# computations/root_digger

Measured on AMD Instinct MI355X. Metric: candidate-root lnL evals/sec, higher is better.
Workload: dtype f64

## Files before the change

### root_digger_amd/csrc/kernels_fused.hip

```cpp
#include <algorithm>
#include <cstdlib>

#include "common.hpp"
#include "expm_k4.hpp"
#include "fused.hpp"

namespace rdamd {

#pragma clang fp contract(off)

__device__ __forceinline__ double pow2_neg256(int d) {
  return d == 0 ? 1.0 : (d == 1 ? kScaleThreshold
       : (d == 2 ? kScaleThreshold * kScaleThreshold
       : (d == 3 ? kScaleThreshold * kScaleThreshold * kScaleThreshold : 0.0)));
}

__device__ __forceinline__ unsigned uni(unsigned x) {
  return (unsigned)__builtin_amdgcn_readfirstlane((int)x);
}

template <int TR>
constexpr unsigned tab_doubles() { return 8u * TR; }

typedef unsigned v2u __attribute__((ext_vector_type(2)));
// ... 503 lines not shown
    const unsigned k3 = kind & 3u;                                                              \
    if (k3 == kFusedTT) {                                                                       \
      if (TR == 16) {                                                                           \
        ((lds_f64_ptr)(size_t)tab_wr)[0] = ex;                                                  \
        ((lds_f64_ptr)(size_t)tab_wr)[4 * TR] = ey;                                             \
      } else {    \
        __builtin_amdgcn_s_waitcnt(0x0f70);                                       \
      }                                                                                         \
      RDAMD_STAMP(1)                                                                            \
      _Pragma("unroll") for (int q = 0; q < NS; ++q) { read_row<0, TR>(rowx[q], tx[q]); read_row<kYSlot, TR>(rowy[q], ty[q]); } \
      RDAMD_LOAD_TIPS(nxt, ncx, ncy, nex, ney) RDAMD_LATE_DESC(cur, idx2)                       \
      RDAMD_STAMP(2)                                                                            \
      if (kind & 0x100u) {           \
        if (kind & 0x200u) {     \
          _Pragma("unroll") for (int q = 0; q < NS; ++q) {                                      \
            matvec(M, st.v[q], s0[q]);                                                          \
            if (!SPEC) s0sc[q] = st.sc[q];                                                      \
          }                                                                                     \
        } else if (RL >= 2 && (kind & 0x800u)) {                   \
          _Pragma("unroll") for (int q = 0; q < NS; ++q) {                                      \
            matvec(M, st.v[q], s1[q]);                                                          \
            if (!SPEC) s1sc[q] = st.sc[q];                                                      \
          }                                                                                     \
        } else {                                                                                \
          _Pragma("unroll") for (int q = 0; q < NS; ++q) {                                      \
            double tp[4];                                                                       \
            matvec(M, st.v[q], tp);                                                             \
            if (SP > 0) {                                                                       \
              stack_push<NS, !SPEC>(sp, kind, q, stk_lds, stksc_lds, spill_off, tp, st.sc[q]);  \
            } else {                                                                            \
              double2 *d = stk + (size_t)(sp * NS + q) * 128;                                   \
              d[0] = make_double2(tp[0], tp[1]);                                                \
              d[64] = make_double2(tp[2], tp[3]);                                               \
              if (!SPEC) stk_sc[(sp * NS + q) * 64] = st.sc[q];                                 \
            }                                                                                   \
          }                                                                                     \
          if (SP == 0 || !(kind & 0x20000u)) ++sp;    \
        }                                                                                       \
      }                                                                                         \
      RDAMD_STAMP(3)                                                                            \
      RDAMD_LOAD_M(nxt, M)                                                                      \
      _Pragma("unroll") for (int q = 0; q < NS; ++q) {                                          \
        st.sc[q] = 0;                                                                           \
        if (tt_safe) { _Pragma("unroll") for (int k = 0; k < 4; ++k) st.v[q][k] = tx[q][k] * ty[q][k]; } \
      }                                                                                         \
      if (!tt_safe) combine_sites<NS>(tx, ty, st.v, st.sc);                                     \
    } else if (k3 == kFusedRT) {                                                                \
      if (TR == 16) ((lds_f64_ptr)(size_t)tab_wr)[4 * TR] = ey;                                 \
      else __builtin_amdgcn_s_waitcnt(0x0f70);             \
      RDAMD_STAMP(1)                                                                            \
      _Pragma("unroll") for (int q = 0; q < NS; ++q) read_row<kYSlot, TR>(rowy[q], ty[q]);      \
      RDAMD_LOAD_TIPS(nxt, ncx, ncy, nex, ney) RDAMD_LATE_DESC(cur, idx2)                       \
      RDAMD_STAMP(2)                                                                            \
      _Pragma("unroll") for (int q = 0; q < NS; ++q) matvec(M, st.v[q], tx[q]);                 \
      RDAMD_STAMP(3)                                                                            \
      RDAMD_LOAD_M(nxt, M)                                                                      \
      combine_sites<NS, kRT>(tx, ty, st.v, st.sc);                                          \
    } else {         \
      if (kind & 0x400u) {           \
        RDAMD_STAMP(1)                                                                          \
        RDAMD_LOAD_TIPS(nxt, ncx, ncy, nex, ney) RDAMD_LATE_DESC(cur, idx2)                     \
        RDAMD_STAMP(2)                                                                          \
        _Pragma("unroll") for (int q = 0; q < NS; ++q) matvec(M, st.v[q], tx[q]);               \
        RDAMD_STAMP(3)                                                                          \
        RDAMD_LOAD_M(nxt, M)                                                                    \
        if (!SPEC) { _Pragma("unroll") for (int q = 0; q < NS; ++q) st.sc[q] += s0sc[q]; }      \
        combine_sites<NS, kRP>(tx, s0, st.v, st.sc);                                                 \
      } else if (RL >= 2 && (kind & 0x1000u)) {                                                 \
        RDAMD_STAMP(1)                                                                          \
        RDAMD_LOAD_TIPS(nxt, ncx, ncy, nex, ney) RDAMD_LATE_DESC(cur, idx2)                     \
        RDAMD_STAMP(2)                                                                          \
        _Pragma("unroll") for (int q = 0; q < NS; ++q) matvec(M, st.v[q], tx[q]);               \
        RDAMD_STAMP(3)                                                                          \
        RDAMD_LOAD_M(nxt, M)                                                                    \
        if (!SPEC) { _Pragma("unroll") for (int q = 0; q < NS; ++q) st.sc[q] += s1sc[q]; }      \
        combine_sites<NS, kRP>(tx, s1, st.v, st.sc);                                                 \
      } else {                                                                                  \
        int scy[NS];                                                                            \
        f64x2_t plo[NS], phi[NS];                                                               \
        if (SP == 0 || !(kind & 0x40000u)) --sp;                                                \
        _Pragma("unroll") for (int q = 0; q < NS; ++q) {                                        \
          if (SP > 0) {          \
            stack_pop_issue<NS, !SPEC>(sp, kind, q, stk_lds, stksc_lds, spill_off, plo[q], phi[q], scy[q]); \
          } else {                                                                              \
            const double2 *d = stk + (size_t)(sp * NS + q) * 128;                               \
            const double2 lo = d[0], hi = d[64];                                                \
            ty[q][0] = lo.x; ty[q][1] = lo.y; ty[q][2] = hi.x; ty[q][3] = hi.y;                 \
            scy[q] = SPEC ? 0 : stk_sc[(sp * NS + q) * 64];                                     \
          }                                                                                     \
        }                                                                                       \
        RDAMD_STAMP(1)                                                                          \
        RDAMD_LOAD_TIPS(nxt, ncx, ncy, nex, ney) RDAMD_LATE_DESC(cur, idx2)                     \
        RDAMD_STAMP(2)                                                                          \
        _Pragma("unroll") for (int q = 0; q < NS; ++q) matvec(M, st.v[q], tx[q]);               \
        RDAMD_STAMP(3)                                                                          \
        RDAMD_LOAD_M(nxt, M)                                                                    \
        if (SP > 0) {                                                                           \
          stack_pop_wait<NS, !SPEC>(plo, phi, scy);                                             \
          _Pragma("unroll") for (int q = 0; q < NS; ++q) {                                      \
            ty[q][0] = plo[q].x; ty[q][1] = plo[q].y; ty[q][2] = phi[q].x; ty[q][3] = phi[q].y; \
          }                                                                                     \
        }                                                                                       \
        if (!SPEC) { _Pragma("unroll") for (int q = 0; q < NS; ++q) st.sc[q] += scy[q]; }       \
        combine_sites<NS, kRP>(tx, ty, st.v, st.sc);                                        \
      }                                                                                         \
    }                                                                                           \
    RDAMD_STAMP(4)                                                                              \
    RDAMD_STAMP_STORE(kind)                                                                     \
    if (EXPORT && (kind & 0x18000u)) {     \
      double *ec = (kind & 0x8000u) ? a.export_clv[0] : a.export_clv[1];                        \
      unsigned *en = (kind & 0x8000u) ? a.export_cnt[0] : a.export_cnt[1];                      \
      _Pragma("unroll") for (int q = 0; q < NS; ++q)                                            \
        if (valid[q]) {                                                                         \
          const size_t at = (size_t)site[q] * R + r;                                            \
          reinterpret_cast<double2 *>(ec + at * 4)[0] = make_double2(st.v[q][0], st.v[q][1]);   \
          reinterpret_cast<double2 *>(ec + at * 4)[1] = make_double2(st.v[q][2], st.v[q][3]);   \
          en[at] = (unsigned)st.sc[q];                                                          \
        }                                                                                       \
    }                                                                                           \
  }

    double s0[NS][4];
    int s0sc[NS];
    double s1[NS][4];
    int s1sc[NS];
#pragma unroll
    for (int q = 0; q < NS; ++q) {
      s0sc[q] = 0;
#pragma unroll
      for (int k = 0; k < 4; ++k) s0[q][k] = 0.0;
    }
#pragma unroll
    for (int q = 0; q < NS; ++q) {
      s1sc[q] = 0;
#pragma unroll
      for (int k = 0; k < 4; ++k) s1[q][k] = 0.0;
    }
    FusedOp dA = load_const(prog);
    FusedOp dB = load_const(prog + 1);
    unsigned cxA[NS], cyA[NS], cxB[NS], cyB[NS];
    double exA = 0.5, eyA = 0.25, exB = 0.5, eyB = 0.25;
#pragma unroll
    for (int q = 0; q < NS; ++q) { cxA[q] = cxB[q] = 1; cyA[q] = cyB[q] = 2; }
    RDAMD_LOAD_TIPS_NOW(dA, cxA, cyA, exA, eyA)
#if defined(RDAMD_ABLATION) && defined(RDAMD_ABL_NOTIPS)
#pragma unroll
    for (int q = 0; q < NS; ++q) { cxB[q] = cxA[q]; cyB[q] = cyA[q]; }
#endif
    double M[16];
    RDAMD_LOAD_M(dA, M)
    unsigned i = 0;
    for (; i + 1 < nops; i += 2) {
      RDAMD_STEP(dA, dB, cxA, cyA, exA, eyA, cxB, cyB, exB, eyB, i + 2)
      RDAMD_STEP(dB, dA, cxB, cyB, exB, eyB, cxA, cyA, exA, eyA, i + 3)
    }
    if (i < nops) {
      RDAMD_STEP(dA, dB, cxA, cyA, exA, eyA, cxB, cyB, exB, eyB, i + 2)
    }
#undef RDAMD_STEP
    const double w = rw[r];
#pragma unroll
    for (int q = 0; q < NS; ++q) {
      double f = __builtin_fma(st.v[q][3], freqs[3],
                               __builtin_fma(st.v[q][2], freqs[2], __builtin_fma(st.v[q][1], freqs[1], st.v[q][0] * freqs[0])));
      f *= w;
      if (RW) {
        term[q] = f;
        smin[q] = st.sc[q];
      } else if (r == 0) {
        term[q] = f;
        smin[q] = st.sc[q];
      } else if (st.sc[q] >= smin[q]) {
        term[q] = __builtin_fma(f, pow2_neg256(st.sc[q] - smin[q]), term[q]);
      } else {
        term[q] = __builtin_fma(term[q], pow2_neg256(smin[q] - st.sc[q]), f);
        smin[q] = st.sc[q];
      }
    }
  }

  if (TR > 16) __builtin_amdgcn_s_waitcnt(0x0f70);
  if (RW) {
    __syncthreads();
    double *xf = lds + (size_t)wave * NS * 64 + lane;
    int *xs = reinterpret_cast<int *>(lds + (size_t)R * NS * 64) + (size_t)wave * NS * 64 + lane;
#pragma unroll
    for (int q = 0; q < NS; ++q) {
      xf[q * 64] = term[q];
      xs[q * 64] = smin[q];
    }
    __syncthreads();
    if (wave != 0u) return;
    for (unsigned r = 1; r < R; ++r) {
      const double *yf = lds + (size_t)r * NS * 64 + lane;
      const int *ys = reinterpret_cast<const int *>(lds + (size_t)R * NS * 64) + (size_t)r * NS * 64 + lane;
#pragma unroll
      for (int q = 0; q < NS; ++q) {
        const double f = yf[q * 64];
        const int sc = ys[q * 64];
        if (sc >= smin[q]) {
          term[q] = __builtin_fma(f, pow2_neg256(sc - smin[q]), term[q]);
        } else {
          term[q] = __builtin_fma(term[q], pow2_neg256(smin[q] - sc), f);
          smin[q] = sc;
        }
      }
    }
  }
  if constexpr (SPEC) {
    bool low = false;
#pragma unroll
    for (int q = 0; q < NS; ++q) low = low || (valid[q] && (unsigned)__double2hiint(term[q]) < 0x07B00000u);
    if (__builtin_amdgcn_ballot_w64(low) != 0ull && lane == 0) {
      const_cast<FusedJob *>(a.jobs)[job].tt_unsafe = 1u;
      *a.any_unsafe = 1u;
    }
  }
#pragma unroll
  for (int q = 0; q < NS; ++q) {
    double l = __builtin_fma((double)smin[q], kLogScaleThreshold, log(term[q]));
    l *= (double)a.pattern_weights[site[q]];
    if (!valid[q]) l = 0.0;
    if (a.persite && valid[q]) a.persite[(size_t)job * S + site[q]] = l;
#pragma unroll
    for (int off = 32; off > 0; off >>= 1) l += __shfl_down(l, off);
    if (lane == 0) a.partials[(size_t)job * (gridDim.x * NS) + bx * NS + q] = l;
  }
}

#pragma clang fp contract(fast)

__global__ void __launch_bounds__(256)
fused_finish_kernel(const double *__restrict__ partials, unsigned per_job,
                    const FusedJob *__restrict__ jobs, unsigned unsafe_pass,
                    double *__restrict__ out, double *__restrict__ host_out,
                    const unsigned *__restrict__ any_unsafe, unsigned *__restrict__ host_flag,
                    double *__restrict__ flag_f64) {
  __shared__ double lds[4];
  if (host_flag && blockIdx.x == 0 && threadIdx.x == 0) *host_flag = *any_unsafe;
  if (flag_f64 && blockIdx.x == 0 && threadIdx.x == 0) *flag_f64 = *any_unsafe ? 1.0 : 0.0;
  if ((jobs[blockIdx.x].tt_unsafe != 0u) != (unsafe_pass != 0u)) return;
  const double *p = partials + (size_t)blockIdx.x * per_job;
  double acc = 0.0;
  for (unsigned i = threadIdx.x; i < per_job; i += 256) acc += p[i];
#pragma unroll
  for (int off = 32; off > 0; off >>= 1) acc += __shfl_down(acc, off);
  if ((threadIdx.x & 63) == 0) lds[threadIdx.x >> 6] = acc;
  __syncthreads();
  if (threadIdx.x == 0) {
    const double v = ((lds[0] + lds[1]) + lds[2]) + lds[3];
    out[blockIdx.x] = v;
    if (host_out) host_out[blockIdx.x] = v;
  }
}

struct ExportFixupArgs {
  double *clv[2];
  const unsigned *cnt[2];
  unsigned *scaler[2];
  unsigned sites, R;
};
__global__ void __launch_bounds__(64)
fused_export_fixup_kernel(ExportFixupArgs x) {
  const unsigned k = blockIdx.y;
  double *__restrict__ clv = x.clv[k];
  const unsigned *__restrict__ cnt = x.cnt[k];
  if (!clv) return;
  const unsigned R = x.R;
  for (unsigned site = blockIdx.x * 1024u + threadIdx.x; site < min(x.sites, (blockIdx.x + 1) * 1024u); site += 64u) {
  unsigned smin = cnt[(size_t)site * R];
  for (unsigned r = 1; r < R; ++r) smin = min(smin, cnt[(size_t)site * R + r]);
  for (unsigned r = 0; r < R; ++r) {
    const unsigned d = cnt[(size_t)site * R + r] - smin;
    if (d) {
      const double f = d < 4u ? pow2_neg256((int)d) : (d == 4u ? 0x1p-1024 : 0.0);
      double *v = clv + ((size_t)site * R + r) * 4;
#pragma unroll
      for (int i = 0; i < 4; ++i) v[i] *= f;
    }
  }
  x.scaler[k][site] = smin;
  }
}

__global__ void __launch_bounds__(64)
fused_finish_wave_kernel(const double *__restrict__ partials, unsigned per_job, double *__restrict__ out,
                         double *__restrict__ host_out) {
  double acc[4] = {0.0, 0.0, 0.0, 0.0};
#pragma unroll
  for (unsigned w = 0; w < 4; ++w)
    for (unsigned i = w * 64u + threadIdx.x; i < per_job; i += 256) acc[w] += partials[i];
#pragma unroll
  for (unsigned w = 0; w < 4; ++w)
#pragma unroll
    for (int off = 32; off > 0; off >>= 1) acc[w] += __shfl_down(acc[w], off);
  if (threadIdx.x == 0) {
    const double v = ((acc[0] + acc[1]) + acc[2]) + acc[3];
    out[0] = v;
    if (host_out) host_out[0] = v;
  }
}

constexpr unsigned kSlimPasses = 16;
__global__ void __launch_bounds__(64)
fused_pmatrix_k4_kernel(const double *__restrict__ q, const double *__restrict__ rates,
                        FusedJob *__restrict__ jobs, unsigned n_jobs,
                        unsigned n_mat, unsigned R, double *__restrict__ pmat,
                        double *__restrict__ tiptab, size_t pmat_job_stride, size_t tiptab_job_stride,
                        unsigned table_rows, unsigned *__restrict__ any_unsafe) {
  const unsigned lane = threadIdx.x, e = lane & 15u;
  const int base = (int)(lane & ~15u);
  const size_t per_job = (size_t)n_mat * R;
  const size_t total = per_job * n_jobs;
  for (unsigned pass = 0; pass < kSlimPasses; ++pass) {
    const size_t first = (size_t)blockIdx.x * (kSlimPasses * 4) + pass * 4;
    if (first >= total) break;
    const size_t gid_raw = first + (lane >> 4);
    const bool live = gid_raw < total;
    const size_t gid = live ? gid_raw : total - 1;
    const unsigned job = (unsigned)(gid / per_job);
    const unsigned rem = (unsigned)(gid % per_job);
    const unsigned m = rem / R, r = rem % R;
    const double t = jobs[job].brlen[m] * rates[(size_t)job * R + r];
    double v = expm_k4_coop16(q + (size_t)job * 16, t);
    v = v <= 0.0 ? 0.0 : v;
    if (live) pmat[(size_t)job * pmat_job_stride + ((size_t)m * R + r) * 16 + e] = v;
    double *tt = tiptab + (size_t)job * tiptab_job_stride + ((size_t)m * R + r) * 64;
#pragma unroll
    for (unsigned k = 0; k < 4; ++k) {
      const unsigned L = e + 16u * k;
      const unsigned c = table_rows > 16 ? (L >> 1) & 15u : L >> 2;
      const unsigned i = table_rows > 16 ? (L >> 5) * 2 + (L & 1u) : L & 3u;
      double acc = 0.0;
#pragma unroll
      for (int j = 0; j < 4; ++j) {
        const double pj = __shfl(v, base + (int)i * 4 + j);
        if ((c >> j) & 1) acc += pj;
      }
      if (live) tt[L] = acc;
    }
    if (live && v > 0.0 && v < 0x1p-128) {
      jobs[job].tt_unsafe = 1u;
      *any_unsafe = 1u;
    }
  }
}

__global__ void __launch_bounds__(64)
fused_pmatrix_k4_wide_kernel(const double *__restrict__ q, const double *__restrict__ rates,
                        FusedJob *__restrict__ jobs, unsigned n_jobs,
                        unsigned n_mat, unsigned R, double *__restrict__ pmat,
                        double *__restrict__ tiptab, size_t pmat_job_stride, size_t tiptab_job_stride,
                        unsigned table_rows, unsigned *__restrict__ any_unsafe) {
  __shared__ double sh[64 * 17];
  __shared__ unsigned long long base_pm[64], base_tt[64];
  const unsigned lane = threadIdx.x;
  const size_t per_job = (size_t)n_mat * R;
  const size_t total = per_job * n_jobs;
  const size_t gid_raw = (size_t)blockIdx.x * blockDim.x + threadIdx.x;
  const bool live = gid_raw < total;
  const size_t gid = live ? gid_raw : total - 1;
  const unsigned job = (unsigned)(gid / per_job);
  const unsigned rem = (unsigned)(gid % per_job);
  const unsigned m = rem / R, r = rem % R;
  const double t = jobs[job].brlen[m] * rates[(size_t)job * R + r];
  const double *qq = q + (size_t)job * 16;
  double out[16];
  expm_k4(qq, t, out);
#pragma unroll
  for (int i = 0; i < 16; ++i) {
    out[i] = out[i] <= 0.0 ? 0.0 : out[i];
    sh[lane * 17 + i] = out[i];
  }
  base_pm[lane] = (unsigned long long)job * pmat_job_stride + ((size_t)m * R + r) * 16;
  base_tt[lane] = (unsigned long long)job * tiptab_job_stride + ((size_t)m * R + r) * 64;
  __syncthreads();
  const unsigned n_live = (unsigned)(total - (size_t)blockIdx.x * 64 < 64 ? total - (size_t)blockIdx.x * 64 : 64);
#pragma unroll 4
  for (unsigned it = 0; it < 16; ++it) {
    const unsigned e = it * 64 + lane, pr = e >> 4, k = e & 15u;
    if (pr < n_live) pmat[base_pm[pr] + k] = sh[pr * 17 + k];
  }
  const unsigned c = table_rows > 16 ? (lane >> 1) & 15u : lane >> 2;
  const unsigned i = table_rows > 16 ? (lane >> 5) * 2 + (lane & 1u) : lane & 3u;
  for (unsigned pr = 0; pr < n_live; ++pr) {
    const double *o = sh + pr * 17 + i * 4;
    double acc = 0.0;
#pragma unroll
    for (int j = 0; j < 4; ++j)
      if ((c >> j) & 1) acc += o[j];
    tiptab[base_tt[pr] + lane] = acc;
  }
  bool tiny = false;
#pragma unroll
  for (int k = 0; k < 16; ++k) tiny = tiny || (out[k] > 0.0 && out[k] < 0x1p-128);
  if (tiny) {
    jobs[job].tt_unsafe = 1u;
    *any_unsafe = 1u;
  }
}

hipError_t launch_fused_pmatrix(const FusedArgs &a, const double *d_q, const double *d_rates,
                                unsigned n_jobs, unsigned n_mat, bool slim, hipStream_t stream) {
  const size_t total = (size_t)n_jobs * n_mat * a.rate_cats;
  if (!total) return hipSuccess;
  if (slim)
    fused_pmatrix_k4_kernel<<<(unsigned)((total + kSlimPasses * 4 - 1) / (kSlimPasses * 4)), 64, 0, stream>>>(
        d_q, d_rates, const_cast<FusedJob *>(a.jobs), n_jobs, n_mat, a.rate_cats, const_cast<double *>(a.pmat),
        const_cast<double *>(a.tiptab), a.pmat_job_stride, a.tiptab_job_stride, a.table_rows, a.any_unsafe);
  else
    fused_pmatrix_k4_wide_kernel<<<(unsigned)((total + 63) / 64), 64, 0, stream>>>(
        d_q, d_rates, const_cast<FusedJob *>(a.jobs), n_jobs, n_mat, a.rate_cats, const_cast<double *>(a.pmat),
        const_cast<double *>(a.tiptab), a.pmat_job_stride, a.tiptab_job_stride, a.table_rows, a.any_unsafe);
  return hipGetLastError();
}

template <int NS, bool TTCHECK, int RL, int TR, bool RW, int SP, bool EXPORT = false, bool SPEC = false>
static hipError_t launch_fused_variant(const FusedArgs &a, unsigned n_jobs, unsigned max_depth, unsigned gx,
                                       hipStream_t stream) {
  const unsigned n_waves = RW ? a.rate_cats : 1u;
  const size_t per_wave = tab_doubles<TR>() * sizeof(double) +
                          (size_t)(SP > 0 || !max_depth ? 1 : max_depth) * NS * 64 * (4 * sizeof(double) + sizeof(int));
  const size_t lds = std::max<size_t>(per_wave * n_waves, (size_t)n_waves * NS * 64 * 12);
  {
    static std::mutex lds_mu;
    static size_t lds_allowed = 48 * 1024;
    std::lock_guard<std::mutex> guard(lds_mu);
    if (lds > lds_allowed) {
      hipError_t e = hipFuncSetAttribute((const void *)fused_dna_eval_kernel<NS, TTCHECK, RL, TR, RW, SP, EXPORT, SPEC>,
                                         hipFuncAttributeMaxDynamicSharedMemorySize, (int)lds);
      if (e != hipSuccess) return e;
      lds_allowed = lds;
    }
  }
  static const bool lds_starts_at_zero = [] {
    hipFuncAttributes attr;
    return hipFuncGetAttributes(&attr, (const void *)fused_dna_eval_kernel<NS, TTCHECK, RL, TR, RW, SP, EXPORT, SPEC>) == hipSuccess &&
           attr.sharedSizeBytes == 0;
  }();
  if (!lds_starts_at_zero) return hipErrorInvalidValue;
  fused_dna_eval_kernel<NS, TTCHECK, RL, TR, RW, SP, EXPORT, SPEC><<<dim3(gx, a.job_major ? (n_jobs + 7u) / 8u * 8u : n_jobs), 64 * n_waves, lds, stream>>>(a);
  return hipGetLastError();
}

template <int NS, bool TTCHECK, int TR>
static hipError_t launch_fused_variant_rl(const FusedArgs &a, unsigned n_jobs, unsigned max_depth, unsigned gx,
                                          unsigned reg_levels, hipStream_t stream) {
#ifdef RDAMD_ABLATION
  static const unsigned spill_min = getenv("RDAMD_FUSED_SPILL_MIN") ? (unsigned)atoi(getenv("RDAMD_FUSED_SPILL_MIN")) : 2u;
#else
  constexpr unsigned spill_min = 2u;
#endif
  const bool spill = TR > 16 && reg_levels < 2 && max_depth >= spill_min && max_depth <= kFusedSpillLevels;
  if (a.rates_across_waves) {
    if (spill) return launch_fused_variant<NS, TTCHECK, 1, TR, true, kFusedSpillLevels>(a, n_jobs, max_depth, gx, stream);
    return reg_levels >= 2 ? launch_fused_variant<NS, TTCHECK, 2, TR, true, 0>(a, n_jobs, max_depth, gx, stream)
                           : launch_fused_variant<NS, TTCHECK, 1, TR, true, 0>(a, n_jobs, max_depth, gx, stream);
  }
  if constexpr (!TTCHECK)
    if (a.speculate) {
      if (spill) return launch_fused_variant<NS, false, 1, TR, false, kFusedSpillLevels, false, true>(a, n_jobs, max_depth, gx, stream);
      return reg_levels >= 2 ? launch_fused_variant<NS, false, 2, TR, false, 0, false, true>(a, n_jobs, max_depth, gx, stream)
                             : launch_fused_variant<NS, false, 1, TR, false, 0, false, true>(a, n_jobs, max_depth, gx, stream);
    }
  if (spill) return launch_fused_variant<NS, TTCHECK, 1, TR, false, kFusedSpillLevels>(a, n_jobs, max_depth, gx, stream);
  return reg_levels >= 2 ? launch_fused_variant<NS, TTCHECK, 2, TR, false, 0>(a, n_jobs, max_depth, gx, stream)
                         : launch_fused_variant<NS, TTCHECK, 1, TR, false, 0>(a, n_jobs, max_depth, gx, stream);
}

template <int NS, int TR>
static hipError_t launch_fused_eval_ns(const FusedArgs &a, unsigned n_jobs, const unsigned max_depth[2],
                                       unsigned blocks_x, const unsigned reg_levels[2], bool unsafe_pass,
                                       double *d_out, double *h_out, unsigned *h_flag, double *flag_f64,
                                       hipStream_t stream) {
  const unsigned gx = (blocks_x + NS - 1) / NS;
  hipError_t e = unsafe_pass ? launch_fused_variant_rl<NS, true, TR>(a, n_jobs, max_depth[1], gx, reg_levels[1], stream)
                             : launch_fused_variant_rl<NS, false, TR>(a, n_jobs, max_depth[0], gx, reg_levels[0], stream);
  if (e != hipSuccess) return e;
  fused_finish_kernel<<<n_jobs, 256, 0, stream>>>(a.partials, gx * NS, a.jobs, unsafe_pass ? 1u : 0u, d_out, h_out, a.any_unsafe, h_flag, flag_f64);
  return hipGetLastError();
}

hipError_t launch_fused_eval(const FusedArgs &a, unsigned n_jobs, const unsigned max_depth[2],
                             unsigned blocks_x, unsigned sites_per_lane, const unsigned reg_levels[2],
                             bool unsafe_pass, double *d_out, double *h_out, unsigned *h_flag, hipStream_t stream,
                             double *flag_f64) {
  if (!n_jobs) return hipSuccess;
  if (a.table_rows > 16)
    return sites_per_lane == 2 ? launch_fused_eval_ns<2, 64>(a, n_jobs, max_depth, blocks_x, reg_levels, unsafe_pass, d_out, h_out, h_flag, flag_f64, stream)
                               : launch_fused_eval_ns<1, 64>(a, n_jobs, max_depth, blocks_x, reg_levels, unsafe_pass, d_out, h_out, h_flag, flag_f64, stream);
  return sites_per_lane == 2 ? launch_fused_eval_ns<2, 16>(a, n_jobs, max_depth, blocks_x, reg_levels, unsafe_pass, d_out, h_out, h_flag, flag_f64, stream)
                             : launch_fused_eval_ns<1, 16>(a, n_jobs, max_depth, blocks_x, reg_levels, unsafe_pass, d_out, h_out, h_flag, flag_f64, stream);
}

hipError_t launch_fused_export(const FusedArgs &a, unsigned max_depth, unsigned blocks_x, unsigned reg_levels,
                               unsigned *const d_scaler[2], double *d_out, double *h_out, hipStream_t stream) {
  if (a.table_rows != 16 || a.rates_across_waves || a.job_major || a.n_jobs != 1) return hipErrorInvalidValue;
  hipError_t e = reg_levels >= 2 ? launch_fused_variant<1, true, 2, 16, false, 0, true>(a, 1, max_depth, blocks_x, stream)
                                 : launch_fused_variant<1, true, 1, 16, false, 0, true>(a, 1, max_depth, blocks_x, stream);
  if (e != hipSuccess) return e;
  fused_finish_wave_kernel<<<1, 64, 0, stream>>>(a.partials, blocks_x, d_out, h_out);
  if (a.export_clv[0] || a.export_clv[1]) {
    ExportFixupArgs x;
    for (int k = 0; k < 2; ++k) { x.clv[k] = a.export_clv[k]; x.cnt[k] = a.export_cnt[k]; x.scaler[k] = d_scaler[k]; }
    x.sites = a.sites; x.R = a.rate_cats;
    fused_export_fixup_kernel<<<dim3((a.sites + 1023u) / 1024u, 2), 64, 0, stream>>>(x);
  }
  return hipGetLastError();
}

}

#if defined(RDAMD_ABLATION) && defined(RDAMD_ABL_STAMPS)
extern "C" int rdamd_abl_stamps_config(unsigned job, unsigned stride) {
  const unsigned cfg[2] = {job, stride};
  void *buf = nullptr;
  if (hipGetSymbolAddress(&buf, HIP_SYMBOL(rdamd::rdamd_stamp_buf)) != hipSuccess) return 0;
  if (hipMemset(buf, 0, sizeof(rdamd::rdamd_stamp_buf)) != hipSuccess) return 0;
  return hipMemcpyToSymbol(HIP_SYMBOL(rdamd::rdamd_stamp_cfg), cfg, sizeof cfg) == hipSuccess;
}
extern "C" int rdamd_abl_stamps_read(unsigned long long *host) {
  if (hipDeviceSynchronize() != hipSuccess) return 0;
  return hipMemcpyFromSymbol(host, HIP_SYMBOL(rdamd::rdamd_stamp_buf), sizeof(rdamd::rdamd_stamp_buf)) == hipSuccess;
}
#endif
```

### root_digger_amd/csrc/schedule_plan.hpp

```cpp
#pragma once

#include <cmath>
#include <cstring>
#include <unordered_map>
#include <vector>

#include "clades.hpp"
#include "fused.hpp"
#include "traversal_compiler.hpp"

namespace rdamd {

using ClvMap = std::unordered_map<unsigned, unsigned>;

struct ScheduleCheck {
  enum Kind { kOk, kEmpty, kOperation, kBranch } kind = kOk;
  unsigned at = 0;
  ClvMap producer;
  std::vector<int> consumer;
  std::vector<double> brlen;
  bool matrix_shared = false;
};

inline ScheduleCheck validate_schedule(unsigned tips, unsigned clv_buffers, unsigned prob_matrices,
                                       const rdamd_operation_t *ops, unsigned n_ops, const unsigned *matrix_indices,
                                       const double *branch_lengths, unsigned n_matrices) {
  ScheduleCheck v;
  if (n_ops == 0) {
    v.kind = ScheduleCheck::kEmpty;
    return v;
  }
  const unsigned nclv = tips + clv_buffers;
  v.consumer.assign(n_ops, -1);
  for (unsigned i = 0; i < n_ops; ++i) {
    const rdamd_operation_t &o = ops[i];
    bool bad = o.parent_clv_index < tips || o.parent_clv_index >= nclv ||
               o.child1_clv_index >= nclv || o.child2_clv_index >= nclv ||
               o.child1_matrix_index >= prob_matrices || o.child2_matrix_index >= prob_matrices;
    for (unsigned ch : {o.child1_clv_index, o.child2_clv_index}) {
      if (ch < tips) continue;
      auto it = v.producer.find(ch);
      if (it == v.producer.end() || v.consumer[it->second] >= 0) bad = true;
      else v.consumer[it->second] = (int)i;
    }
    if (v.producer.count(o.parent_clv_index)) bad = true;
    if (bad) {
      v.kind = ScheduleCheck::kOperation;
      v.at = i;
      return v;
    }
    v.producer[o.parent_clv_index] = i;
  }
  v.brlen.assign(prob_matrices, 0.0);
  for (unsigned m = 0; m < n_matrices; ++m) {
    if (matrix_indices[m] >= prob_matrices || !(branch_lengths[m] >= 0.0) || !std::isfinite(branch_lengths[m])) {
      v.kind = ScheduleCheck::kBranch;
      v.at = m;
      return v;
    }
    v.brlen[matrix_indices[m]] = branch_lengths[m];
  }
  std::vector<unsigned char> uses(prob_matrices, 0);
  for (unsigned i = 0; i < n_ops; ++i)
    for (unsigned m : {ops[i].child1_matrix_index, ops[i].child2_matrix_index})
      if (uses[m]++) v.matrix_shared = true;
  return v;
}

struct ScheduleShape {
  unsigned tips = 0, sites = 0, tip_stride = 0, rate_cats = 0, prob_matrices = 0;
  bool k20 = false;
  bool wide_mode = false;
};

struct Program {
  std::vector<FusedOp> steps;
  unsigned depth = 1, reg_levels = 1, matvecs = 0;
};

struct ProgramTrace {
  Compiler c;
  unsigned runner_up = 0;
};

inline unsigned compile_program(const ScheduleShape &sh, const std::vector<rdamd_operation_t> &list,
                                const ClvMap &pseudo_row, const ClvMap &pseudo_wide, Program &out,
                                ProgramTrace *trace = nullptr) {
  Compiler local;
  Compiler &c = trace ? trace->c : local;
  const bool k20 = sh.k20, wide_mode = sh.wide_mode;
  c.ops = list.data(); c.n_ops = (unsigned)list.size(); c.tips = sh.tips; c.sites = sh.sites;
  c.tip_stride = sh.tip_stride * (wide_mode ? 2u : 1u); c.rate_cats = sh.rate_cats;
  c.unit = sh.rate_cats * (k20 ? 3200u : 128u);
  c.split_park = k20;
  c.pseudo_row = pseudo_row;
  c.pseudo_wide = pseudo_wide;
  c.wide_base = 8u * sh.prob_matrices * sh.rate_cats * 16u;
  c.dma_offsets = !k20 && wide_mode;
  c.place_parks = !k20 && wide_mode;
  {
    const rdamd_operation_t &root = list.back();
    if (root.child1_clv_index >= sh.tips) c.mark_clv[0] = root.child1_clv_index;
    if (root.child2_clv_index >= sh.tips) c.mark_clv[1] = root.child2_clv_index;
  }
  for (unsigned i = 0; i < c.n_ops; ++i) c.producer[list[i].parent_clv_index] = i;
  c.need.assign(c.n_ops, 0);
  c.compute_need(c.n_ops - 1);
  c.out.reserve(c.n_ops);
  c.emit(c.n_ops - 1, false, 0);
  const unsigned runner_up = c.place_levels(k20 ? 0u : (wide_mode ? 1u + kFusedSpillLevels : 3u), kFusedSpillLevels - 1u);
  if (trace) trace->runner_up = runner_up;
  size_t n_real = 0;
  for (const FusedOp &f : c.out)
    if (!c.split_park || (f.flags & 3u) != kFusedPark) ++n_real;
  if (n_real != c.n_ops) return (unsigned)(c.n_ops - n_real);
  out.depth = !c.park_class.empty() ? 1u + c.mem_depth
                                    : std::max(1u, c.max_depth > c.reg_levels ? c.max_depth - c.reg_levels : 0);
  out.reg_levels = c.reg_levels;
  out.matvecs = c.matvecs;
  if (trace) out.steps = c.out;
  else out.steps = std::move(c.out);
  return 0;
}

struct CladeSelection {
  std::vector<char> small;
  std::vector<CladeStep> steps;
  std::vector<CladeGroup> groups;
  std::vector<unsigned> tip_ops;
  ClvMap pseudo_wide;
  unsigned n_wide = 0, clade_rows = 0;
  std::vector<rdamd_operation_t> kept(const rdamd_operation_t *ops) const {
    std::vector<rdamd_operation_t> list;
    for (size_t i = 0; i < small.size(); ++i)
      if (!small[i]) list.push_back(ops[i]);
    return list;
  }
};

inline CladeSelection select_clades(const rdamd_operation_t *ops, unsigned n_ops, unsigned tips, const ScheduleCheck &v,
                                    const std::vector<unsigned> &node_id, const std::vector<unsigned> &n_classes,
                                    unsigned class_limit) {
  CladeSelection sel;
  sel.small.assign(n_ops, 0);
  for (unsigned i = 0; i + 1 < n_ops; ++i)
    sel.small[i] = !v.matrix_shared && n_classes[i] > 0 && n_classes[i] <= class_limit;
  auto mat_above = [&](unsigned i) {
    const rdamd_operation_t &c = ops[v.consumer[i]];
    return c.child1_clv_index == ops[i].parent_clv_index ? c.child1_matrix_index : c.child2_matrix_index;
  };
  for (unsigned i = 0; i + 1 < n_ops; ++i) {
    if (!sel.small[i] || sel.small[v.consumer[i]]) continue;
    CladeGroup g;
    g.first = (unsigned)sel.steps.size();
    auto walk = [&](auto &&self, unsigned j) -> unsigned {
      const rdamd_operation_t &o = ops[j];
      CladeStep st;
      memset(&st, 0, sizeof st);
      const unsigned ch[2] = {o.child1_clv_index, o.child2_clv_index};
      const unsigned mt[2] = {o.child1_matrix_index, o.child2_matrix_index};
      for (int k = 0; k < 2; ++k)
        st.src[k] = ch[k] < tips ? mt[k] : (0x80000000u | self(self, v.producer.at(ch[k])));
      st.n_classes = n_classes[j];
      st.out_mat = mat_above(j);
      st.last = j == i ? 1u : 0u;
      st.wide_slot = 0xffffffffu;
      if (j == i && n_classes[j] > 16) {
        st.wide_slot = sel.n_wide;
        sel.pseudo_wide[o.parent_clv_index] = sel.n_wide++;
      }
      st.pad = node_id[j];
      sel.clade_rows += n_classes[j];
      sel.steps.push_back(st);
      return (unsigned)sel.steps.size() - 1 - g.first;
    };
    walk(walk, i);
    g.count = (unsigned)sel.steps.size() - g.first;
    sel.groups.push_back(g);
    sel.tip_ops.push_back(i);
  }
  return sel;
}

struct ScheduleBlock {
  size_t o_prog = 0, o_plain = 0, o_steps = 0, o_groups = 0, o_brlen = 0, o_tipmask = 0, total = 0;
  std::vector<char> host;
};

inline ScheduleBlock pack_schedule_block(const Program &main_prog, const Program *plain, const std::vector<CladeStep> &steps,
                                         const std::vector<CladeGroup> &groups, const std::vector<double> &brlen,
                                         bool k20, unsigned tips, const rdamd_operation_t *ops, unsigned n_ops) {
  constexpr size_t kTail = 4;
  auto up = [](size_t b) { return (b + 63) & ~(size_t)63; };
  const size_t n_main = main_prog.steps.size() + kTail, n_plain = plain ? plain->steps.size() + kTail : 0;
  const size_t prob_matrices = brlen.size();
  ScheduleBlock b;
  b.o_plain = up(b.o_prog + sizeof(FusedOp) * n_main);
  b.o_steps = up(b.o_plain + sizeof(FusedOp) * n_plain);
  b.o_groups = up(b.o_steps + sizeof(CladeStep) * steps.size());
  b.o_brlen = up(b.o_groups + sizeof(CladeGroup) * groups.size());
  b.o_tipmask = up(b.o_brlen + sizeof(double) * prob_matrices);
  b.total = up(b.o_tipmask + (k20 ? sizeof(uint32_t) * ((prob_matrices + 31) / 32) : 0));
  b.host.assign(b.total, 0);
  auto put_program = [&](size_t at, const Program &pr) {
    FusedOp *dst = (FusedOp *)(b.host.data() + at);
    memcpy(dst, pr.steps.data(), sizeof(FusedOp) * pr.steps.size());
    for (size_t k = 0; k < kTail; ++k) dst[pr.steps.size() + k] = pr.steps.back();
  };
  put_program(b.o_prog, main_prog);
  if (plain) put_program(b.o_plain, *plain);
  if (!steps.empty()) memcpy(b.host.data() + b.o_steps, steps.data(), sizeof(CladeStep) * steps.size());
  if (!groups.empty()) memcpy(b.host.data() + b.o_groups, groups.data(), sizeof(CladeGroup) * groups.size());
  if (prob_matrices) memcpy(b.host.data() + b.o_brlen, brlen.data(), sizeof(double) * prob_matrices);
  if (k20) {
    uint32_t *mask = (uint32_t *)(b.host.data() + b.o_tipmask);
    for (unsigned i = 0; i < n_ops; ++i) {
      if (ops[i].child1_clv_index < tips) mask[ops[i].child1_matrix_index >> 5] |= 1u << (ops[i].child1_matrix_index & 31u);
      if (ops[i].child2_clv_index < tips) mask[ops[i].child2_matrix_index >> 5] |= 1u << (ops[i].child2_matrix_index & 31u);
    }
  }
  return b;
}

}
```

### root_digger_amd/csrc/traversal_compiler.hpp

```cpp
#pragma once

#include <algorithm>
#include <cstring>
#include <unordered_map>
#include <vector>

#include "../../include/root_digger_amd.h"
#include "fused.hpp"

namespace rdamd {

struct Compiler {
  const rdamd_operation_t *ops;
  unsigned n_ops, tips, sites, tip_stride, rate_cats;
  unsigned unit = 0;
  bool split_park = false;
  unsigned reg_levels = 1;
  unsigned reg_level = 0;
  std::unordered_map<unsigned, unsigned> producer;
  std::unordered_map<unsigned, unsigned> pseudo_row;
  std::unordered_map<unsigned, unsigned> pseudo_wide;
  unsigned wide_base = 0;
  bool dma_offsets = false;
  unsigned mark_clv[2] = {~0u, ~0u};
  unsigned matvecs = 0;
  std::vector<unsigned> need;
  std::vector<FusedOp> out;
  unsigned depth = 0, max_depth = 0;
  unsigned parks_at[16] = {0};
  bool ok = true;
  bool place_parks = false;
  std::vector<unsigned char> park_class;
  unsigned mem_now = 0, mem_depth = 0;
  std::vector<int> place_memo;

  bool is_inner(unsigned clv) const { return clv >= tips && !pseudo_row.count(clv); }
  unsigned row_of(unsigned clv) const { return clv < tips ? clv : pseudo_row.at(clv); }

  unsigned compute_need(unsigned i) {
    const rdamd_operation_t &o = ops[i];
    unsigned n1 = 0, n2 = 0;
    const bool i1 = is_inner(o.child1_clv_index), i2 = is_inner(o.child2_clv_index);
    if (i1) n1 = compute_need(producer.at(o.child1_clv_index));
    if (i2) n2 = compute_need(producer.at(o.child2_clv_index));
    unsigned r;
    if (i1 && i2) r = std::max(std::max(n1, n2), std::min(n1, n2) + 1);
    else r = i1 ? n1 : (i2 ? n2 : 0);
    need[i] = r;
    return r;
  }

  void emit(unsigned i, bool live, unsigned park_mat, unsigned park_cls = 0) {
    const rdamd_operation_t &o = ops[i];
    const bool i1 = is_inner(o.child1_clv_index), i2 = is_inner(o.child2_clv_index);
    FusedOp f;
    memset(&f, 0, sizeof(f));
    unsigned matM = 0, matX = 0, matY = 0, kind = 0, spill = 0, tipX_row = 0, tipY_row = 0, placed = 0;
    if (!i1 && !i2) {
      kind = kFusedTT;
      spill = live ? 1 : 0;
      tipX_row = row_of(o.child1_clv_index); matX = o.child1_matrix_index;
      tipY_row = row_of(o.child2_clv_index); matY = o.child2_matrix_index;
      if (live) {
        matM = park_mat;
        if (park_cls) {
          if (park_cls == 1) spill |= 2;
          else if (park_cls == 2) placed = 0x20000u;
          else mem_depth = std::max(mem_depth, ++mem_now);
        } else if (reg_levels >= 2) {
          if (depth == 0) spill |= 2;
          else if (depth == 1) spill |= 8;
        } else if (depth == reg_level) {
          spill |= 2;
        }
        ++parks_at[depth < 15 ? depth : 15];
        ++depth;
        max_depth = std::max(max_depth, depth);
        if (split_park) {
          FusedOp park;
          memset(&park, 0, sizeof(park));
          park.pM = matM * unit;
          park.flags = kFusedPark | ((spill & 2) ? 0x200u : 0u);
          out.push_back(park);
          matM = 0;
          spill = 0;
        }
      }
    } else if (i1 != i2) {
      const bool first_inner = i1;
      emit(producer.at(first_inner ? o.child1_clv_index : o.child2_clv_index), live, park_mat, park_cls);
      kind = kFusedRT;
      matM = first_inner ? o.child1_matrix_index : o.child2_matrix_index;
      tipY_row = row_of(first_inner ? o.child2_clv_index : o.child1_clv_index);
      matY = first_inner ? o.child2_matrix_index : o.child1_matrix_index;
    } else {
      const unsigned a = producer.at(o.child1_clv_index), b = producer.at(o.child2_clv_index);
      const bool a_first = need[a] >= need[b];
      const unsigned first = a_first ? a : b, second = a_first ? b : a;
      const unsigned mat_first = a_first ? o.child1_matrix_index : o.child2_matrix_index;
      const unsigned mine = park_class.empty() ? 0u : park_class[i];
      emit(first, live, park_mat, park_cls);
      emit(second, true, mat_first, mine);
      kind = kFusedRP;
      matM = a_first ? o.child2_matrix_index : o.child1_matrix_index;
      --depth;
      if (mine) {
        if (mine == 1) spill |= 4;
        else if (mine == 2) placed = 0x40000u;
        else --mem_now;
      } else if (reg_levels >= 2) {
        if (depth == 0) spill |= 4;
        else if (depth == 1) spill |= 16;
      } else if (depth == reg_level) {
        spill |= 4;
      }
    }
    matvecs += (i1 ? 1u : 0u) + (i2 ? 1u : 0u);
    f.pM = matM * unit;
    f.tX = matX * unit;
    f.tY = matY * unit;
    unsigned wide_flags = 0;
    if (kind == kFusedTT || kind == kFusedRT) {
      const unsigned leafX = o.child1_clv_index;
      const unsigned leafY = kind == kFusedTT ? o.child2_clv_index : (i1 ? o.child2_clv_index : o.child1_clv_index);
      if (kind == kFusedTT && pseudo_wide.count(leafX)) {
        f.tX = wide_base + pseudo_wide.at(leafX) * rate_cats * 512u;
        wide_flags |= 0x2000u;
      }
      if (pseudo_wide.count(leafY)) {
        f.tY = wide_base + pseudo_wide.at(leafY) * rate_cats * 512u;
        wide_flags |= 0x4000u;
      }
    }
    f.pad[0] = matX * rate_cats * (kFused20TabDoubles * 8u);
    f.pad[1] = matY * rate_cats * (kFused20TabDoubles * 8u);
    if (dma_offsets) {
      f.pad[0] = f.tX * 4u + kFusedDmaBias;
      f.pad[1] = f.tY * 4u + kFusedDmaBias - kFusedDmaYSlot;
    }
    f.cX = tipX_row * tip_stride;
    f.cY = tipY_row * tip_stride;
    f.flags = kind | (spill << 8) | wide_flags | placed;
    if (o.parent_clv_index == mark_clv[0]) f.flags |= 0x8000u;
    if (o.parent_clv_index == mark_clv[1]) f.flags |= 0x10000u;
    out.push_back(f);
  }
  int place_value(unsigned i, unsigned free_slots) {
    int &memo = place_memo[4 * i + free_slots];
    if (memo >= 0) return memo;
    const rdamd_operation_t &o = ops[i];
    const bool i1 = is_inner(o.child1_clv_index), i2 = is_inner(o.child2_clv_index);
    int v = 0;
    if (i1 != i2) {
      v = place_value(producer.at(i1 ? o.child1_clv_index : o.child2_clv_index), free_slots);
    } else if (i1 && i2) {
      const unsigned a = producer.at(o.child1_clv_index), b = producer.at(o.child2_clv_index);
      const bool a_first = need[a] >= need[b];
      const unsigned first = a_first ? a : b, second = a_first ? b : a;
      const int base = place_value(first, free_slots);
      v = base + place_value(second, free_slots);
      if (free_slots & 1u) v = std::max(v, base + 1025 + place_value(second, free_slots & ~1u));
      if (free_slots & 2u) v = std::max(v, base + 1024 + place_value(second, free_slots & ~2u));
    }
    return memo = v;
  }
  void place_assign(unsigned i, unsigned free_slots) {
    const rdamd_operation_t &o = ops[i];
    const bool i1 = is_inner(o.child1_clv_index), i2 = is_inner(o.child2_clv_index);
    if (i1 != i2) {
      place_assign(producer.at(i1 ? o.child1_clv_index : o.child2_clv_index), free_slots);
    } else if (i1 && i2) {
      const unsigned a = producer.at(o.child1_clv_index), b = producer.at(o.child2_clv_index);
      const bool a_first = need[a] >= need[b];
      const unsigned first = a_first ? a : b, second = a_first ? b : a;
      const int base = place_value(first, free_slots), v = place_value(i, free_slots);
      unsigned cls = 3, left = free_slots;
      if ((free_slots & 1u) && v == base + 1025 + place_value(second, free_slots & ~1u)) { cls = 1; left = free_slots & ~1u; }
      else if ((free_slots & 2u) && v == base + 1024 + place_value(second, free_slots & ~2u)) { cls = 2; left = free_slots & ~2u; }
      park_class[i] = (unsigned char)cls;
      place_assign(first, free_slots);
      place_assign(second, left);
    }
  }
  unsigned place_levels(unsigned two_reg_beyond, unsigned mem_limit = 0) {
    const bool two_reg = two_reg_beyond > 0 && max_depth > two_reg_beyond;
    if (!two_reg && max_depth < 2) return 0;
    bool again = false;
    if (place_parks && !two_reg) {
      place_memo.assign((size_t)4 * n_ops, -1);
      park_class.assign(n_ops, 0);
      place_value(n_ops - 1, 3u);
      place_assign(n_ops - 1, 3u);
      out.clear();
      depth = max_depth = mem_now = mem_depth = 0;
      matvecs = 0;
      memset(parks_at, 0, sizeof parks_at);
      emit(n_ops - 1, false, 0);
      if (mem_depth <= mem_limit) return 0;
      park_class.clear();
      mem_now = mem_depth = 0;
      again = true;
    }
    unsigned busiest = 0;
    for (unsigned l = 1; l < max_depth && l < 16; ++l)
      if (parks_at[l] > parks_at[busiest]) busiest = l;
    unsigned second = busiest == 0 ? 1 : 0;
    for (unsigned l = 0; l < max_depth && l < 16; ++l)
      if (l != busiest && parks_at[l] > parks_at[second]) second = l;
    if (two_reg || busiest != 0 || again) {
      out.clear();
      depth = max_depth = 0;
      matvecs = 0;
      memset(parks_at, 0, sizeof parks_at);
      if (two_reg) reg_levels = 2;
      else reg_level = busiest;
      emit(n_ops - 1, false, 0);
    }
    return two_reg ? 0u : second - (second > busiest ? 1u : 0u);
  }
};

}
```

Before: 89130.

## Skip writing unused P-matrices and tip tables via per-matrix read masks

The traversal compiler now records which probability matrices are read as full P-matrices and which as tip lookup tables. These bitmasks are packed after the branch lengths in the schedule block, and the pmatrix kernels store only the outputs that are actually consumed. The wide kernel uses ballots and readlane to iterate just over the wanted entries. This cuts global stores in the pmatrix stage, at the cost of extra mask reads and the risk of stale data if a reader is missed. The mask is not written on the k20 path, yet the kernels read it unconditionally.

```diff
diff --git a/root_digger_amd/csrc/kernels_fused.hip b/root_digger_amd/csrc/kernels_fused.hip
--- a/root_digger_amd/csrc/kernels_fused.hip
+++ b/root_digger_amd/csrc/kernels_fused.hip
@@ -829,6 +829,11 @@
 }
 
 constexpr unsigned kSlimPasses = 16;
+__device__ __forceinline__ unsigned front_reads(const double *brlen, unsigned n_mat, unsigned m) {
+  const unsigned *mask = reinterpret_cast<const unsigned *>(brlen + n_mat);
+  const unsigned nw = (n_mat + 31u) >> 5, w = m >> 5, b = m & 31u;
+  return ((mask[w] >> b) & 1u) | (((mask[nw + w] >> b) & 1u) << 1);
+}
 __global__ void __launch_bounds__(64)
 fused_pmatrix_k4_kernel(const double *__restrict__ q, const double *__restrict__ rates,
                         FusedJob *__restrict__ jobs, unsigned n_jobs,
@@ -848,10 +853,12 @@
     const unsigned job = (unsigned)(gid / per_job);
     const unsigned rem = (unsigned)(gid % per_job);
     const unsigned m = rem / R, r = rem % R;
-    const double t = jobs[job].brlen[m] * rates[(size_t)job * R + r];
+    const double *brlen = jobs[job].brlen;
+    const unsigned reads = live ? front_reads(brlen, n_mat, m) : 0u;
+    const double t = brlen[m] * rates[(size_t)job * R + r];
     double v = expm_k4_coop16(q + (size_t)job * 16, t);
     v = v <= 0.0 ? 0.0 : v;
-    if (live) pmat[(size_t)job * pmat_job_stride + ((size_t)m * R + r) * 16 + e] = v;
+    if (reads & 1u) pmat[(size_t)job * pmat_job_stride + ((size_t)m * R + r) * 16 + e] = v;
     double *tt = tiptab + (size_t)job * tiptab_job_stride + ((size_t)m * R + r) * 64;
 #pragma unroll
     for (unsigned k = 0; k < 4; ++k) {
@@ -864,9 +871,9 @@
         const double pj = __shfl(v, base + (int)i * 4 + j);
         if ((c >> j) & 1) acc += pj;
       }
-      if (live) tt[L] = acc;
-    }
-    if (live && v > 0.0 && v < 0x1p-128) {
+      if (reads & 2u) tt[L] = acc;
+    }
+    if ((reads & 2u) && v > 0.0 && v < 0x1p-128) {
       jobs[job].tt_unsafe = 1u;
       *any_unsafe = 1u;
     }
@@ -880,7 +887,7 @@
                         double *__restrict__ tiptab, size_t pmat_job_stride, size_t tiptab_job_stride,
                         unsigned table_rows, unsigned *__restrict__ any_unsafe) {
   __shared__ double sh[64 * 17];
-  __shared__ unsigned long long base_pm[64], base_tt[64];
+  __shared__ unsigned long long base_pm[64];
   const unsigned lane = threadIdx.x;
   const size_t per_job = (size_t)n_mat * R;
   const size_t total = per_job * n_jobs;
@@ -890,7 +897,9 @@
   const unsigned job = (unsigned)(gid / per_job);
   const unsigned rem = (unsigned)(gid % per_job);
   const unsigned m = rem / R, r = rem % R;
-  const double t = jobs[job].brlen[m] * rates[(size_t)job * R + r];
+  const double *brlen = jobs[job].brlen;
+  const unsigned reads = front_reads(brlen, n_mat, m);
+  const double t = brlen[m] * rates[(size_t)job * R + r];
   const double *qq = q + (size_t)job * 16;
   double out[16];
   expm_k4(qq, t, out);
@@ -900,28 +909,37 @@
     sh[lane * 17 + i] = out[i];
   }
   base_pm[lane] = (unsigned long long)job * pmat_job_stride + ((size_t)m * R + r) * 16;
-  base_tt[lane] = (unsigned long long)job * tiptab_job_stride + ((size_t)m * R + r) * 64;
+  const unsigned long long my_tt = (unsigned long long)job * tiptab_job_stride + ((size_t)m * R + r) * 64;
   __syncthreads();
-  const unsigned n_live = (unsigned)(total - (size_t)blockIdx.x * 64 < 64 ? total - (size_t)blockIdx.x * 64 : 64);
-#pragma unroll 4
+  const unsigned long long want_p = __ballot(live && (reads & 1u)), want_t = __ballot(live && (reads & 2u));
   for (unsigned it = 0; it < 16; ++it) {
-    const unsigned e = it * 64 + lane, pr = e >> 4, k = e & 15u;
-    if (pr < n_live) pmat[base_pm[pr] + k] = sh[pr * 17 + k];
+    if (!((want_p >> (it * 4u)) & 0xfull)) continue;
+    const unsigned pr = it * 4u + (lane >> 4), k = lane & 15u;
+    if ((want_p >> pr) & 1ull) pmat[base_pm[pr] + k] = sh[pr * 17 + k];
   }
   const unsigned c = table_rows > 16 ? (lane >> 1) & 15u : lane >> 2;
   const unsigned i = table_rows > 16 ? (lane >> 5) * 2 + (lane & 1u) : lane & 3u;
-  for (unsigned pr = 0; pr < n_live; ++pr) {
+  auto entry = [&](unsigned pr) {
     const double *o = sh + pr * 17 + i * 4;
     double acc = 0.0;
 #pragma unroll
     for (int j = 0; j < 4; ++j)
       if ((c >> j) & 1) acc += o[j];
-    tiptab[base_tt[pr] + lane] = acc;
+    return acc;
+  };
+  auto table_of = [&](unsigned pr) {
+    const unsigned lo = (unsigned)__builtin_amdgcn_readlane((int)(unsigned)my_tt, (int)pr);
+    const unsigned hi = (unsigned)__builtin_amdgcn_readlane((int)(unsigned)(my_tt >> 32), (int)pr);
+    return tiptab + (((unsigned long long)hi << 32) | lo) + lane;
+  };
+  for (unsigned long long todo = want_t; todo; todo &= todo - 1) {
+    const unsigned pr = (unsigned)__builtin_ctzll(todo);
+    *table_of(pr) = entry(pr);
   }
   bool tiny = false;
 #pragma unroll
   for (int k = 0; k < 16; ++k) tiny = tiny || (out[k] > 0.0 && out[k] < 0x1p-128);
-  if (tiny) {
+  if (tiny && live && (reads & 2u)) {
     jobs[job].tt_unsafe = 1u;
     *any_unsafe = 1u;
   }
diff --git a/root_digger_amd/csrc/schedule_plan.hpp b/root_digger_amd/csrc/schedule_plan.hpp
--- a/root_digger_amd/csrc/schedule_plan.hpp
+++ b/root_digger_amd/csrc/schedule_plan.hpp
@@ -76,6 +76,7 @@
 struct Program {
   std::vector<FusedOp> steps;
   unsigned depth = 1, reg_levels = 1, matvecs = 0;
+  std::vector<uint32_t> reads_p, reads_tab;
 };
 
 struct ProgramTrace {
@@ -118,6 +119,8 @@
                                     : std::max(1u, c.max_depth > c.reg_levels ? c.max_depth - c.reg_levels : 0);
   out.reg_levels = c.reg_levels;
   out.matvecs = c.matvecs;
+  out.reads_p = c.reads_p;
+  out.reads_tab = c.reads_tab;
   if (trace) out.steps = c.out;
   else out.steps = std::move(c.out);
   return 0;
@@ -182,8 +185,35 @@
   return sel;
 }
 
+struct ReadMasks {
+  std::vector<uint32_t> p, tab;
+};
+
+inline ReadMasks read_masks(const Program &main_prog, const Program *plain, const std::vector<CladeStep> &steps,
+                            size_t prob_matrices) {
+  ReadMasks r;
+  const size_t nw = (prob_matrices + 31) / 32;
+  r.p.assign(nw, 0u);
+  r.tab.assign(nw, 0u);
+  auto add = [&](std::vector<uint32_t> &to, const std::vector<uint32_t> &from) {
+    for (size_t w = 0; w < from.size() && w < nw; ++w) to[w] |= from[w];
+  };
+  for (const Program *pr : {&main_prog, plain}) {
+    if (!pr) continue;
+    add(r.p, pr->reads_p);
+    add(r.tab, pr->reads_tab);
+  }
+  for (const CladeStep &st : steps) {
+    for (int k = 0; k < 2; ++k)
+      if (!(st.src[k] & 0x80000000u)) r.tab[st.src[k] >> 5] |= 1u << (st.src[k] & 31u);
+    r.p[st.out_mat >> 5] |= 1u << (st.out_mat & 31u);
+  }
+  return r;
+}
+
 struct ScheduleBlock {
   size_t o_prog = 0, o_plain = 0, o_steps = 0, o_groups = 0, o_brlen = 0, o_tipmask = 0, total = 0;
+  size_t o_masks = 0;
   std::vector<char> host;
 };
 
@@ -199,7 +229,9 @@
   b.o_steps = up(b.o_plain + sizeof(FusedOp) * n_plain);
   b.o_groups = up(b.o_steps + sizeof(CladeStep) * steps.size());
   b.o_brlen = up(b.o_groups + sizeof(CladeGroup) * groups.size());
-  b.o_tipmask = up(b.o_brlen + sizeof(double) * prob_matrices);
+  const size_t mask_words = (prob_matrices + 31) / 32;
+  b.o_masks = b.o_brlen + sizeof(double) * prob_matrices;
+  b.o_tipmask = up(b.o_masks + (k20 ? 0 : sizeof(uint32_t) * 2 * mask_words));
   b.total = up(b.o_tipmask + (k20 ? sizeof(uint32_t) * ((prob_matrices + 31) / 32) : 0));
   b.host.assign(b.total, 0);
   auto put_program = [&](size_t at, const Program &pr) {
@@ -212,6 +244,11 @@
   if (!steps.empty()) memcpy(b.host.data() + b.o_steps, steps.data(), sizeof(CladeStep) * steps.size());
   if (!groups.empty()) memcpy(b.host.data() + b.o_groups, groups.data(), sizeof(CladeGroup) * groups.size());
   if (prob_matrices) memcpy(b.host.data() + b.o_brlen, brlen.data(), sizeof(double) * prob_matrices);
+  if (!k20 && prob_matrices) {
+    const ReadMasks r = read_masks(main_prog, plain, steps, prob_matrices);
+    memcpy(b.host.data() + b.o_masks, r.p.data(), sizeof(uint32_t) * mask_words);
+    memcpy(b.host.data() + b.o_masks + sizeof(uint32_t) * mask_words, r.tab.data(), sizeof(uint32_t) * mask_words);
+  }
   if (k20) {
     uint32_t *mask = (uint32_t *)(b.host.data() + b.o_tipmask);
     for (unsigned i = 0; i < n_ops; ++i) {
diff --git a/root_digger_amd/csrc/traversal_compiler.hpp b/root_digger_amd/csrc/traversal_compiler.hpp
--- a/root_digger_amd/csrc/traversal_compiler.hpp
+++ b/root_digger_amd/csrc/traversal_compiler.hpp
@@ -26,6 +26,11 @@
   unsigned matvecs = 0;
   std::vector<unsigned> need;
   std::vector<FusedOp> out;
+  std::vector<uint32_t> reads_p, reads_tab;
+  static void mark_read(std::vector<uint32_t> &mask, unsigned m) {
+    if (mask.size() <= (m >> 5)) mask.resize((m >> 5) + 1, 0u);
+    mask[m >> 5] |= 1u << (m & 31u);
+  }
   unsigned depth = 0, max_depth = 0;
   unsigned parks_at[16] = {0};
   bool ok = true;
@@ -63,6 +68,7 @@
       tipY_row = row_of(o.child2_clv_index); matY = o.child2_matrix_index;
       if (live) {
         matM = park_mat;
+        mark_read(reads_p, park_mat);
         if (park_cls) {
           if (park_cls == 1) spill |= 2;
           else if (park_cls == 2) placed = 0x20000u;
@@ -93,6 +99,7 @@
       matM = first_inner ? o.child1_matrix_index : o.child2_matrix_index;
       tipY_row = row_of(first_inner ? o.child2_clv_index : o.child1_clv_index);
       matY = first_inner ? o.child2_matrix_index : o.child1_matrix_index;
+      mark_read(reads_p, matM);
     } else {
       const unsigned a = producer.at(o.child1_clv_index), b = producer.at(o.child2_clv_index);
       const bool a_first = need[a] >= need[b];
@@ -103,6 +110,7 @@
       emit(second, true, mat_first, mine);
       kind = kFusedRP;
       matM = a_first ? o.child2_matrix_index : o.child1_matrix_index;
+      mark_read(reads_p, matM);
       --depth;
       if (mine) {
         if (mine == 1) spill |= 4;
@@ -132,6 +140,8 @@
         wide_flags |= 0x4000u;
       }
     }
+    if (kind == kFusedTT && !(wide_flags & 0x2000u)) mark_read(reads_tab, matX);
+    if (kind != kFusedRP && !(wide_flags & 0x4000u)) mark_read(reads_tab, matY);
     f.pad[0] = matX * rate_cats * (kFused20TabDoubles * 8u);
     f.pad[1] = matY * rate_cats * (kFused20TabDoubles * 8u);
     if (dma_offsets) {
```

Result: no change. 88440 (-0.8%).
